# neptune-ai/open-solution-salt-identification

Hardware: AMD Instinct MI355X
Metric: training images/sec, U-Net ResNet34 101x101 (pad->128) bs32/GPU (higher is better)
Workload: dtype bf16; 1 GPU; architectures.unet.UNetResNet(34, hypercolumn) 128x128 (101 resized+edge-padded) batch 32/GPU, lovasz loss, Adam lr1e-4 L2 1e-4, train-mode BN; global_batch=32, parallelism=dp1

## Files before the change

open-solution-salt-identification_amd/csrc/conv_ws.hip:

```cpp
#include <type_traits>
#include "common.h"

#ifndef SALT_LS_D1
#define SALT_LS_D1 4
#endif
#ifndef SALT_LS_NLW
#define SALT_LS_NLW 4
#endif
#ifndef SALT_LS_PREFETCH
#define SALT_LS_PREFETCH 1
#endif
#ifndef SALT_LS_ABLATE
#define SALT_LS_ABLATE 0
#endif
#ifndef SALT_WS_CLK
#define SALT_WS_CLK 0
#endif

namespace {

struct WsKP {
    const bf16_t* x; const bf16_t* w; bf16_t* y;
    const float* bias; const float* scale; const float* shift;
    int B, H, W, x_cs, y_cs, OH, OW;
    int yH, yW, fold_top, ox_shift;
    int Cout, n_tiles, slots;
    int tiles_x, tiles_y, ntiles, per_xcd;
    int min_dy, min_dx, pad_mode;
    int tap_off[9];
    int relu, accumulate;
    const bf16_t* bnb_y; const bf16_t* bnb_a; int bnb_cs, bnb_acs, bnb_relu;
    const float* bnb_mean; const float* bnb_invstd; const float* bnb_gamma; const float* bnb_beta;
    double* fin_acc;
    double* bnb_acc;
    const bf16_t* res; int res_cs;
    long long y_plane;
};

__device__ __attribute__((aligned(16))) unsigned int g_ws_zero[4] = {0u, 0u, 0u, 0u};
#if SALT_WS_CLK
__device__ unsigned long long g_ws_clk[256 * 48];
#endif

typedef __attribute__((address_space(3))) void* lds_ptr_t;
typedef const __attribute__((address_space(1))) void* glb_ptr_t;

__device__ __forceinline__ int ws_swz(int row, int slot) { return row * 64 + (((slot ^ (row >> 2)) & 3) << 4); }
__device__ __forceinline__ int ws_perm(int m) { return (int)((0x73261540u >> ((m >> 2) * 4)) & 0xfu) * 4 + (m & 3); }

__device__ __forceinline__ int ws_perm_inv(int q) { return (int)((0x74216530u >> ((q >> 2) * 4)) & 0xfu) * 4 + (q & 3); }

template <int N> __device__ __forceinline__ void ws_wait_vm() {
    asm volatile("s_waitcnt vmcnt(%0)" :: "n"(N) : "memory");
}

template <int N, int S> __device__ __forceinline__ void ws_halve(float* v, int l31) {
    const bool up = (l31 >> S) & 1;
#pragma unroll
    for (int i = 0; i < N / 2; ++i) {
        const float keep = up ? v[i + N / 2] : v[i], give = up ? v[i] : v[i + N / 2];
        v[i] = keep + __shfl_xor(give, 1 << S);
    }
}

struct WsEpi {
    bf16_t* y; const bf16_t* bnb_y; const bf16_t* bnb_a;
    int y_cs, bnb_cs, bnb_acs, relu, accumulate, bnb_relu;
    bool has_affine, sums;
    const bf16_t* res; int res_cs;
};
template <int NI> struct WsOps { u32x4 oldv[2][NI][2], yv[2][NI][2], av[2][NI][2]; };
template <int NI, bool OLD>
__device__ __forceinline__ void ws_prefetch_operands(const WsEpi& p, const unsigned (&pix)[2], int n0, int khalf, WsOps<NI>& o) {
#pragma unroll
    for (int j = 0; j < NI; ++j)
#pragma unroll
        for (int i = 0; i < 2; ++i)
#pragma unroll
            for (int gp = 0; gp < 2; ++gp) {
                const unsigned c = n0 + 8 * khalf + 32 * j + 16 * gp;
                if (OLD && p.accumulate) o.oldv[i][j][gp] = *reinterpret_cast<const u32x4*>(p.y + (pix[i] * (unsigned)p.y_cs + c));
                if (OLD && p.res) o.oldv[i][j][gp] = *reinterpret_cast<const u32x4*>(p.res + (pix[i] * (unsigned)p.res_cs + c));
                if (p.sums) {
                    o.yv[i][j][gp] = *reinterpret_cast<const u32x4*>(p.bnb_y + (pix[i] * (unsigned)p.bnb_cs + c));
                    if (p.bnb_a) o.av[i][j][gp] = *reinterpret_cast<const u32x4*>(p.bnb_a + (pix[i] * (unsigned)p.bnb_acs + c));
                }
            }
}

struct WsLaneGeo {
    bool valid[2];
    bool do_right, do_top;
    bool fr_on, ft_on;
    int fr_src0, fr_src1;
    int ft_src0, ft_src1;
};

template <int NI, int MODE, bool FOLD>
__device__ __forceinline__ void ws_epilogue_tile(const WsEpi& p, f32x16 (&acc)[2][NI], const unsigned (&pix)[2], const WsLaneGeo& geo, int n0,
                                                 const float* cst, float (&rs0)[NI][4], float (&rs1)[NI][4], int khalf, int l31,
                                                 const WsOps<NI>* pre = nullptr, bool pre_old = true) {
    typedef bf16_t T;
    constexpr int MI = 2, BN = 32 * NI;
    typedef const __attribute__((address_space(3))) float* cst_lds_t;
    cst_lds_t cst_l = (cst_lds_t)cst + 8 * khalf;
    if (MODE == 2) asm volatile("" : "+v"(cst_l));
#pragma unroll
    for (int j = 0; j < NI; ++j) {
        u32x4 oldv[MI][2], yv[MI][2], av[MI][2];
        auto load_operands = [&](int i) {
            if (!geo.valid[i]) return;
            if (pre) {
#pragma unroll
                for (int gp = 0; gp < 2; ++gp) {
                    if (pre_old) oldv[i][gp] = pre->oldv[i][j][gp];
                    else if (p.accumulate) oldv[i][gp] = *reinterpret_cast<const u32x4*>(p.y + (pix[i] * (unsigned)p.y_cs + n0 + 8 * khalf + 32 * j + 16 * gp));
                    yv[i][gp] = pre->yv[i][j][gp]; av[i][gp] = pre->av[i][j][gp];
                }
                return;
            }
            if (MODE != 1 && p.accumulate) {
#pragma unroll
                for (int gp = 0; gp < 2; ++gp)
                    oldv[i][gp] = *reinterpret_cast<const u32x4*>(p.y + (pix[i] * (unsigned)p.y_cs + n0 + 8 * khalf + 32 * j + 16 * gp));
            }
            if (MODE == 0 && p.res) {
#pragma unroll
                for (int gp = 0; gp < 2; ++gp)
                    oldv[i][gp] = *reinterpret_cast<const u32x4*>(p.res + (pix[i] * (unsigned)p.res_cs + n0 + 8 * khalf + 32 * j + 16 * gp));
            }
            if (MODE == 2 && p.sums) {
#pragma unroll
                for (int gp = 0; gp < 2; ++gp) {
                    yv[i][gp] = *reinterpret_cast<const u32x4*>(p.bnb_y + (pix[i] * (unsigned)p.bnb_cs + n0 + 8 * khalf + 32 * j + 16 * gp));
                    if (p.bnb_a) av[i][gp] = *reinterpret_cast<const u32x4*>(p.bnb_a + (pix[i] * (unsigned)p.bnb_acs + n0 + 8 * khalf + 32 * j + 16 * gp));
                }
            }
        };
        if (!FOLD) {
#pragma unroll
            for (int i = 0; i < MI; ++i) load_operands(i);
        }
        float v[MI][16];
#pragma unroll
        for (int i = 0; i < MI; ++i) {
#pragma unroll
            for (int r = 0; r < 16; ++r) v[i][r] = acc[i][j][r];
            if (MODE != 2 && p.has_affine) {
#pragma unroll
                for (int q = 0; q < 4; ++q) {
                    const int ch0 = 32 * j + 8 * q + 4 * khalf;
                    const f32x4 bi = *reinterpret_cast<const f32x4*>(cst + ch0), sc = *reinterpret_cast<const f32x4*>(cst + BN + ch0),
                                sh = *reinterpret_cast<const f32x4*>(cst + 2 * BN + ch0);
#pragma unroll
                    for (int e = 0; e < 4; ++e) {
                        float t = (v[i][4 * q + e] + bi[e]) * sc[e] + sh[e];
                        if (p.relu && !(MODE == 0 && p.res)) t = fmaxf(t, 0.f);
                        v[i][4 * q + e] = t;
                    }
                }
            }
        }
        if (FOLD) {
            const int hb = khalf << 5;
            if (geo.do_right) {
#pragma unroll
                for (int i = 0; i < MI; ++i)
#pragma unroll
                    for (int r = 0; r < 16; ++r) {
                        const float add = __shfl(v[i][r], hb + geo.fr_src0) + __shfl(v[i][r], hb + geo.fr_src1);
                        if (geo.fr_on) v[i][r] += add;
                    }
            }
            if (geo.do_top) {
#pragma unroll
                for (int r = 0; r < 16; ++r) {
                    const float add = __shfl(v[0][r], hb + geo.ft_src0) + __shfl(v[0][r], hb + geo.ft_src1);
                    if (geo.ft_on) v[1][r] += add;
                }
            }
        }
        float t0[16], t1[16];
#pragma unroll
        for (int e = 0; e < 16; ++e) { t0[e] = 0.f; t1[e] = 0.f; }
#pragma unroll
        for (int i = 0; i < MI; ++i) {
            const unsigned yo = pix[i] * (unsigned)p.y_cs + n0 + 8 * khalf + 32 * j;
            if (FOLD) load_operands(i);
            if (MODE == 1) {
#pragma unroll
                for (int r = 0; r < 16; ++r) { t0[r] += v[i][r]; t1[r] += v[i][r] * v[i][r]; }
            }
#pragma unroll
            for (int gp = 0; gp < 2; ++gp) {
                const unsigned ax = f2bf_pk(v[i][8 * gp + 0], v[i][8 * gp + 1]), ay = f2bf_pk(v[i][8 * gp + 2], v[i][8 * gp + 3]);
                const unsigned bx = f2bf_pk(v[i][8 * gp + 4], v[i][8 * gp + 5]), by = f2bf_pk(v[i][8 * gp + 6], v[i][8 * gp + 7]);
                const auto rx = __builtin_amdgcn_permlane32_swap(ax, bx, false, false);
                const auto ry = __builtin_amdgcn_permlane32_swap(ay, by, false, false);
                u32x4 stored = {rx[0], ry[0], rx[1], ry[1]};
                if (!geo.valid[i]) continue;
                if (MODE != 1 && p.accumulate) {
                    float f8[8], o8[8];
                    unpack16<T>(stored, f8); unpack16<T>(oldv[i][gp], o8);
#pragma unroll
                    for (int e = 0; e < 8; ++e) f8[e] += o8[e];
                    stored = pack16<T>(f8);
                }
                if (MODE == 0 && p.res) {
                    float f8[8], o8[8];
                    unpack16<T>(stored, f8); unpack16<T>(oldv[i][gp], o8);
#pragma unroll
                    for (int e = 0; e < 8; ++e) { f8[e] += o8[e]; if (p.relu) f8[e] = fmaxf(f8[e], 0.f); }
                    stored = pack16<T>(f8);
                }
                *reinterpret_cast<u32x4*>(p.y + (yo + 16 * gp)) = stored;
                if (MODE == 2 && p.sums) {
                    const int ch0 = 32 * j + 16 * gp;
                    const cst_lds_t cl = cst_l;
                    float mu[8], is[8], gq[8], yc[8];
                    *reinterpret_cast<f32x4*>(mu) = *reinterpret_cast<const __attribute__((address_space(3))) f32x4*>(cl + ch0);
                    *reinterpret_cast<f32x4*>(mu + 4) = *reinterpret_cast<const __attribute__((address_space(3))) f32x4*>(cl + ch0 + 4);
                    *reinterpret_cast<f32x4*>(is) = *reinterpret_cast<const __attribute__((address_space(3))) f32x4*>(cl + BN + ch0);
                    *reinterpret_cast<f32x4*>(is + 4) = *reinterpret_cast<const __attribute__((address_space(3))) f32x4*>(cl + BN + ch0 + 4);
                    unpack16<T>(stored, gq); unpack16<T>(yv[i][gp], yc);
                    if (p.bnb_a) {
                        float a8[8];
                        unpack16<T>(av[i][gp], a8);
#pragma unroll
                        for (int e = 0; e < 8; ++e) {
                            const float gg = (!p.bnb_relu || a8[e] > 0.f) ? gq[e] : 0.f;
                            t0[gp * 8 + e] += gg; t1[gp * 8 + e] += gg * (yc[e] - mu[e]) * is[e];
                        }
                    } else {
                        float ks[8], sh[8];
                        *reinterpret_cast<f32x4*>(ks) = *reinterpret_cast<const __attribute__((address_space(3))) f32x4*>(cl + 2 * BN + ch0);
                        *reinterpret_cast<f32x4*>(ks + 4) = *reinterpret_cast<const __attribute__((address_space(3))) f32x4*>(cl + 2 * BN + ch0 + 4);
                        *reinterpret_cast<f32x4*>(sh) = *reinterpret_cast<const __attribute__((address_space(3))) f32x4*>(cl + 3 * BN + ch0);
                        *reinterpret_cast<f32x4*>(sh + 4) = *reinterpret_cast<const __attribute__((address_space(3))) f32x4*>(cl + 3 * BN + ch0 + 4);
#pragma unroll
                        for (int e = 0; e < 8; ++e) {
                            const float gg = (!p.bnb_relu || yc[e] * ks[e] + sh[e] > 0.f) ? gq[e] : 0.f;
                            t0[gp * 8 + e] += gg; t1[gp * 8 + e] += gg * (yc[e] - mu[e]) * is[e];
                        }
                    }
                }
            }
        }
        if (MODE != 0 && p.sums) {
            ws_halve<16, 0>(t0, l31); ws_halve<8, 1>(t0, l31);
            ws_halve<16, 0>(t1, l31); ws_halve<8, 1>(t1, l31);
#pragma unroll
            for (int e = 0; e < 4; ++e) { rs0[j][e] += t0[e]; rs1[j][e] += t1[e]; }
        }
    }
}

template <int NI, int MODE, int NW>
__device__ __forceinline__ void ws_sums_flush(float (&rs0)[NI][4], float (&rs1)[NI][4], bool holder, int hw, float* red, int n0, int C,
                                              double* fin_acc, double* bnb_acc, double count, int khalf, int l31) {
    constexpr int BN = 32 * NI;
    const int tid = threadIdx.x;
    const int idx = 8 * (l31 & 1) + 4 * ((l31 >> 1) & 1) + 2 * ((l31 >> 2) & 1) + ((l31 >> 3) & 1);
    if (holder) {
#pragma unroll
        for (int j = 0; j < NI; ++j) {
            ws_halve<4, 2>(rs0[j], l31); ws_halve<2, 3>(rs0[j], l31);
            ws_halve<4, 2>(rs1[j], l31); ws_halve<2, 3>(rs1[j], l31);
            const float s0 = rs0[j][0] + __shfl_xor(rs0[j][0], 16), s1 = rs1[j][0] + __shfl_xor(rs1[j][0], 16);
            const int ch = MODE == 1 ? 32 * j + (idx & 3) + 8 * (idx >> 2) + 4 * khalf : 32 * j + 16 * (idx >> 3) + 8 * khalf + (idx & 7);
            red[(hw * 2 + 0) * BN + ch] = s0;
            red[(hw * 2 + 1) * BN + ch] = s1;
        }
    }
    __syncthreads();
    if (tid < 2 * BN) {
        const int st = tid / BN, n = tid - st * BN;
        double t = 0.0;
#pragma unroll
        for (int w = 0; w < NW; ++w) t += (double)red[(w * 2 + st) * BN + n];
        if (MODE == 1) {
            double* a = fin_acc + (blockIdx.x & 7) * (2 * C + 1);
            fin_add(a + st * C + n0 + n, t);
            if (tid == 0 && count > 0.0) fin_add(a + 2 * C, count);
        } else {
            fin_add(bnb_acc + ((blockIdx.x & 7) * 2 + st) * C + n0 + n, t);
        }
    }
}

template <int NCH, int NI, int MODE, bool FOLD>
__global__ __launch_bounds__(512) void conv_ws_kernel(WsKP p) {
    typedef bf16_t T;
    constexpr int BN = 32 * NI, NT = 9, MI = 2;
    constexpr int HPC = 21;
    constexpr int HP = NCH * HPC;
    constexpr int WP = NCH * NT * BN / 16;
    constexpr int NSW = (WP + 7) / 8;
    constexpr int NSH = (HP + 3) / 4;
    constexpr int W_BYTES = WP * 1024, H_BYTES = HP * 1024, HC_BYTES = HPC * 1024;
    constexpr int OFF_H = W_BYTES, OFF_DUMMY = OFF_H + 2 * H_BYTES;
    constexpr int OFF_CONST = OFF_DUMMY + 1024;
    extern __shared__ __attribute__((aligned(16))) unsigned char smem[];

    const int tid = threadIdx.x, lane = tid & 63;
    const int wave = __builtin_amdgcn_readfirstlane(tid >> 6);
    const int grp = wave >> 2, wm = wave & 3;
    const int khalf = lane >> 5, l31 = lane & 31;

    const int xcd = blockIdx.x & 7, jwg = blockIdx.x >> 3;
    const int nt = jwg % p.n_tiles, slot = jwg / p.n_tiles, n0 = nt * BN;
    const int t_lo = xcd * p.per_xcd;
    const int t_hi = min(t_lo + p.per_xcd, p.ntiles);
    const int n_my = (t_lo + slot < t_hi) ? (t_hi - t_lo - slot + p.slots - 1) / p.slots : 0;
    if (n_my <= 0) return;
    auto tile_of = [&](int k) { return t_lo + slot + k * p.slots; };
    struct TC { int b, oy0, ox0; };
    auto coords = [&](int t) {
        TC c; const int tx = t % p.tiles_x; const int r = t / p.tiles_x;
        c.ox0 = (tx << 4) - p.ox_shift; c.oy0 = (r % p.tiles_y) << 4; c.b = r / p.tiles_y; return c;
    };
#if SALT_WS_CLK
    unsigned long long clk[24]; int nclk = 0;
    auto stamp = [&]() { if (nclk < 22) clk[nclk++] = __builtin_readcyclecounter(); };
#else
    auto stamp = [&]() {};
#endif
    stamp();

    const unsigned char* zp = reinterpret_cast<const unsigned char*>(g_ws_zero);
    auto dma = [&](const void* src, int dst) {
        __builtin_amdgcn_global_load_lds((glb_ptr_t)src, (lds_ptr_t)(smem + dst), 16, 0, 0);
    };
    auto issue_weights = [&]() {
#pragma unroll
        for (int i = 0; i < NSW; ++i) {
            const int q = wave + 8 * i;
            const bool real = q < WP;
            const int R = q * 16 + (lane >> 2);
            const int ct = R / BN, n = R - ct * BN;
            const int cslot = (lane ^ (R >> 2)) & 3;
            const unsigned char* src = real ? reinterpret_cast<const unsigned char*>(p.w + ((ct * p.Cout + n0 + n) * 32 + cslot * 8)) : zp;
            dma(src, real ? q * 1024 : OFF_DUMMY);
        }
    };
    auto issue_halo = [&](const TC& c, int g) {
        int ln = lane;
        asm volatile("" : "+v"(ln));
        const T* xb = p.x + (int64_t)c.b * p.H * p.W * p.x_cs;
        const int iy0 = c.oy0 + p.min_dy, ix0 = c.ox0 + p.min_dx;
        const bool clamp = p.pad_mode != 0;
#pragma unroll
        for (int i = 0; i < NSH; ++i) {
            const int pidx = wm + 4 * i;
            const bool real = pidx < HP;
            const int ch = (NCH > 1 && pidx >= HPC) ? 1 : 0;
            const int row = (pidx - ch * HPC) * 16 + (ln >> 2);
            const int hy = (int)__umulhi((unsigned)row, 238609295u);
            const int hx = row - hy * 18;
            const int iy = iy0 + hy, ix = ix0 + hx;
            const int iyc = min(max(iy, 0), p.H - 1), ixc = min(max(ix, 0), p.W - 1);
            const bool inside = ((unsigned)iy < (unsigned)p.H) & ((unsigned)ix < (unsigned)p.W);
            const bool valid = real & (row < 324) & (clamp | inside);
            const int slot = (ln ^ (row >> 2)) & 3;
            const unsigned char* src = reinterpret_cast<const unsigned char*>(xb + ((iyc * p.W + ixc) * p.x_cs + ch * 32 + slot * 8));
            dma(valid ? src : zp, real ? OFF_H + g * H_BYTES + pidx * 1024 : OFF_DUMMY);
        }
    };

    issue_weights();
    if (grp < n_my) issue_halo(coords(tile_of(grp)), grp);
    if (tid < BN) {
        float* sc = reinterpret_cast<float*>(smem + OFF_CONST);
        if (MODE == 2) {
            if (p.bnb_acc) {
                const float mu = p.bnb_mean[n0 + tid], is = p.bnb_invstd[n0 + tid], k = p.bnb_gamma[n0 + tid] * is;
                sc[tid] = mu; sc[BN + tid] = is; sc[2 * BN + tid] = k; sc[3 * BN + tid] = p.bnb_beta[n0 + tid] - mu * k;
            }
        } else {
            sc[tid] = p.bias ? p.bias[n0 + tid] : 0.f; sc[BN + tid] = p.scale ? p.scale[n0 + tid] : 1.f; sc[2 * BN + tid] = p.shift ? p.shift[n0 + tid] : 0.f;
        }
    }

    int pbase[MI];
#pragma unroll
    for (int i = 0; i < MI; ++i) {
        const int m = wm * 64 + i * 32 + ws_perm(l31);
        pbase[i] = (m >> 4) * 18 + (m & 15);
    }
    f32x16 acc[MI][NI];
    struct Frag { u32x4 a[MI], b[NI]; };
    auto mma_tile = [&](int g) {
        const unsigned char* hb = smem + OFF_H + g * H_BYTES;
        int a_addr[NT][MI], b_addr[NI];
#pragma unroll
        for (int i = 0; i < MI; ++i) {
            int pb = pbase[i];
            asm volatile("" : "+v"(pb));
#pragma unroll
            for (int t = 0; t < NT; ++t) a_addr[t][i] = ws_swz(pb + p.tap_off[t], khalf);
        }
        {
            int lb = l31;
            asm volatile("" : "+v"(lb));
#pragma unroll
            for (int j = 0; j < NI; ++j) b_addr[j] = ws_swz(j * 32 + lb, khalf);
        }
#pragma unroll
        for (int i = 0; i < MI; ++i)
#pragma unroll
            for (int j = 0; j < NI; ++j)
#pragma unroll
                for (int r = 0; r < 16; ++r) acc[i][j][r] = 0.f;
        auto load_frag = [&](int s, Frag& f) {
            const int c = s / (2 * NT), t = (s % (2 * NT)) >> 1, hx = (s & 1) << 5;
#pragma unroll
            for (int i = 0; i < MI; ++i) f.a[i] = *reinterpret_cast<const u32x4*>(hb + c * HC_BYTES + (a_addr[t][i] ^ hx));
#pragma unroll
            for (int j = 0; j < NI; ++j) f.b[j] = *reinterpret_cast<const u32x4*>(smem + (c * NT + t) * (BN * 64) + (b_addr[j] ^ hx));
        };
        auto mma_frag = [&](const Frag& f) {
#pragma unroll
            for (int i = 0; i < MI; ++i)
#pragma unroll
                for (int j = 0; j < NI; ++j)
                    acc[i][j] = __builtin_amdgcn_mfma_f32_32x32x16_bf16(__builtin_bit_cast(bf16x8, f.b[j]), __builtin_bit_cast(bf16x8, f.a[i]), acc[i][j], 0, 0, 0);
        };
        constexpr int NST = NCH * NT * 2;
        Frag f[3];
        load_frag(0, f[0]);
        load_frag(1, f[1]);
        __builtin_amdgcn_sched_group_barrier(0x100, 2 * (MI + NI), 0);
#pragma unroll
        for (int s = 0; s < NST; ++s) {
            if (s + 2 < NST) load_frag(s + 2, f[(s + 2) % 3]);
            mma_frag(f[s % 3]);
            if (s + 2 < NST) __builtin_amdgcn_sched_group_barrier(0x100, MI + NI, 0);
            __builtin_amdgcn_sched_group_barrier(0x008, MI * NI, 0);
        }
    };

    float rs0[NI][4], rs1[NI][4];
#pragma unroll
    for (int j = 0; j < NI; ++j)
#pragma unroll
        for (int e = 0; e < 4; ++e) { rs0[j][e] = 0.f; rs1[j][e] = 0.f; }
    const bool sums = (MODE == 1 && p.fin_acc) || (MODE == 2 && p.bnb_acc);
    const WsEpi ep = {p.y_plane ? p.y + ((long long)nt * p.y_plane - n0) : p.y, p.bnb_y, p.bnb_a, p.y_cs, p.bnb_cs, p.bnb_acs, p.relu, p.accumulate, p.bnb_relu,
                      p.bias || p.scale || p.shift || p.relu, sums, p.res, p.res_cs};

    auto epilogue = [&](const TC& c, int g, bool has_next, const TC& next) {
        unsigned pix[MI];
        WsLaneGeo geo = {{true, true}, false, false, false, false, 0, 0, 0, 0};
#pragma unroll
        for (int i = 0; i < MI; ++i) {
            const int m = wm * 64 + i * 32 + ws_perm(l31);
            const int oy = c.oy0 + (m >> 4), ox = c.ox0 + (m & 15);
            const int iy = oy - p.fold_top;
            geo.valid[i] = ((unsigned)iy < (unsigned)p.yH) & ((unsigned)ox < (unsigned)p.yW);
            pix[i] = (unsigned)((c.b * p.yH + iy) * p.yW + ox);
        }
        if (FOLD) {
            const int q = ws_perm(l31), rs = q >> 4, col = q & 15;
            geo.fr_src0 = ws_perm_inv(rs * 16 + 14); geo.fr_src1 = ws_perm_inv(rs * 16 + 15);
            geo.ft_src0 = ws_perm_inv(col); geo.ft_src1 = ws_perm_inv(16 + col);
            geo.do_right = c.ox0 + 16 == p.OW;
            geo.do_top = wm == 0 && c.oy0 == 0;
            geo.fr_on = col == 13 && geo.do_right;
            geo.ft_on = rs == 0 && geo.do_top;
        }
        ws_epilogue_tile<NI, MODE, FOLD>(ep, acc, pix, geo, n0, reinterpret_cast<const float*>(smem + OFF_CONST), rs0, rs1, khalf, l31);
        stamp();
        if (has_next) {
            __builtin_amdgcn_sched_barrier(0);
            issue_halo(next, g);
        }
    };

    for (int k = 0; k <= n_my; ++k) {
        const int g_mma = k & 1;
        if (k == 0) { if (grp == 0 || n_my < 2) ws_wait_vm<0>(); else ws_wait_vm<NSH>(); }
        else if (grp == g_mma && k < n_my) ws_wait_vm<0>();
        asm volatile("s_waitcnt lgkmcnt(0)" ::: "memory");
        __builtin_amdgcn_s_barrier();
        asm volatile("" ::: "memory");
        stamp();
        if (grp == g_mma) {
            if (k < n_my) { __builtin_amdgcn_s_setprio(1); mma_tile(g_mma); __builtin_amdgcn_s_setprio(0); }
        } else if (k >= 1) {
            const bool has_next = k + 1 < n_my;
            const TC cur = coords(tile_of(k - 1));
            const TC nxt = has_next ? coords(tile_of(k + 1)) : cur;
            epilogue(cur, grp, has_next, nxt);
        }
        stamp();
    }

    if (MODE != 0 && sums) {
        asm volatile("s_waitcnt vmcnt(0)" ::: "memory");
        __syncthreads();
        ws_sums_flush<NI, MODE, 8>(rs0, rs1, true, wave, reinterpret_cast<float*>(smem), n0, p.Cout, p.fin_acc, p.bnb_acc,
                                   nt == 0 ? (double)n_my * 256.0 : 0.0, khalf, l31);
    }
#if SALT_WS_CLK
    if (lane == 0 && (wave == 0 || wave == 4) && blockIdx.x < 256) {
        unsigned long long* o = g_ws_clk + (blockIdx.x * 2 + grp) * 24;
        for (int i = 0; i < 22; ++i) o[i] = i < nclk ? clk[i] : 0ull;
        o[22] = (unsigned long long)n_my;
        o[23] = __builtin_readcyclecounter();
    }
#endif
}


int ws_cus() {
    static int cus = 0;
    if (!cus) {
        hipDeviceProp_t pr; int dev = 0;
        if (hipGetDevice(&dev) == hipSuccess && hipGetDeviceProperties(&pr, dev) == hipSuccess) cus = pr.multiProcessorCount;
        if (cus < 8) cus = 256;
    }
    return cus;
}

template <int NCH, int NI, int MODE, bool FOLD>
int ws_launch_mode(const WsKP& k, hipStream_t st) {
    constexpr int BN = 32 * NI, HP = NCH * 21, WP = NCH * 9 * BN / 16;
    constexpr int LDS = WP * 1024 + 2 * HP * 1024 + 1024 + 4 * BN * 4;
    static_assert(LDS <= 160 * 1024 && 8 * 2 * BN * 4 <= WP * 1024, "LDS budget");
    return salt_launch(conv_ws_kernel<NCH, NI, MODE, FOLD>, dim3((unsigned)(k.slots * k.n_tiles * 8)), dim3(512), LDS, st, k);
}

template <int NCH, int NI>
int ws_launch(const WsKP& k, hipStream_t st) {
    const bool fold = k.fold_top != 0;
    if (k.fin_acc) return ws_launch_mode<NCH, NI, 1, false>(k, st);
    if (k.bnb_acc) return fold ? ws_launch_mode<NCH, NI, 2, true>(k, st) : ws_launch_mode<NCH, NI, 2, false>(k, st);
    return fold ? ws_launch_mode<NCH, NI, 0, true>(k, st) : ws_launch_mode<NCH, NI, 0, false>(k, st);
}

struct LsKP {
    const bf16_t* x; const bf16_t* w; bf16_t* y;
    const float* bias; const float* scale; const float* shift;
    int B, H, W, x_cs, y_cs, OH, OW, Cout;
    int tiles_x, tiles_y, ntiles, per_xcd, n_tiles, slots, nchunk;
    int min_dy, min_dx, pad_mode;
    int tap_off[9];
    int relu, accumulate;
    const bf16_t* bnb_y; const bf16_t* bnb_a; int bnb_cs, bnb_acs, bnb_relu;
    const float* bnb_mean; const float* bnb_invstd; const float* bnb_gamma; const float* bnb_beta;
    double* fin_acc; double* bnb_acc;
    const bf16_t* res; int res_cs;
    long long x_plane;
};

template <int NI, int MODE, int NLW = SALT_LS_NLW, int MT = 1>
__global__ __launch_bounds__(256 + 64 * NLW) void conv_ls_kernel(LsKP p) {
    typedef bf16_t T;
    constexpr int BN = 32 * NI, NT = 9, MI = 2;
    constexpr int HPC = 21, WPC = NT * BN / 16, PC = MT * HPC + WPC;
    constexpr int NS = (PC + NLW - 1) / NLW;
    constexpr int D = NI == 1 ? SALT_LS_D1 : 2;
    constexpr int HT_BYTES = HPC * 1024, H_BYTES = MT * HT_BYTES, CH_BYTES = PC * 1024;
    static_assert(MT == 1 || (MODE == 0 && NI == 2), "two-tile items: plain epilogue, 64-channel blocks");
    constexpr int OFF_DUMMY = D * CH_BYTES, OFF_CONST = OFF_DUMMY + 1024;
    static_assert(OFF_CONST + 4 * BN * 4 <= 160 * 1024, "LDS budget");
    extern __shared__ __attribute__((aligned(16))) unsigned char smem[];

    const int tid = threadIdx.x, lane = tid & 63;
    const int wave = __builtin_amdgcn_readfirstlane(tid >> 6);
    const bool loader = wave >= 4;
    const int wm = wave & 3;
    const int lw = wave - 4;
    const int khalf = lane >> 5, l31 = lane & 31;

    const int xcd = blockIdx.x & 7, jwg = blockIdx.x >> 3;
    if (jwg >= p.slots * p.n_tiles) return;
    const int nt = jwg % p.n_tiles, slot = jwg / p.n_tiles, n0 = nt * BN;
    const int t_lo = xcd * p.per_xcd;
    const int t_hi = min(t_lo + p.per_xcd, p.ntiles);
    const int n_my = (t_lo + slot < t_hi) ? (t_hi - t_lo - slot + p.slots - 1) / p.slots : 0;
    const int n_items = (n_my + MT - 1) / MT;
    if (n_items <= 0) return;
    const int G = n_items * p.nchunk;
    struct TC { int b, oy0, ox0; };
    auto coords = [&](int k) {
        const int t = t_lo + slot + k * p.slots;
        TC c; const int tx = t % p.tiles_x; const int r = t / p.tiles_x;
        c.ox0 = tx << 4; c.oy0 = (r % p.tiles_y) << 4; c.b = r / p.tiles_y; return c;
    };
    if (tid < BN) {
        float* sc = reinterpret_cast<float*>(smem + OFF_CONST);
        if (MODE == 2) {
            if (p.bnb_acc) {
                const float mu = p.bnb_mean[n0 + tid], is = p.bnb_invstd[n0 + tid], k = p.bnb_gamma[n0 + tid] * is;
                sc[tid] = mu; sc[BN + tid] = is; sc[2 * BN + tid] = k; sc[3 * BN + tid] = p.bnb_beta[n0 + tid] - mu * k;
            }
        } else {
            sc[tid] = p.bias ? p.bias[n0 + tid] : 0.f; sc[BN + tid] = p.scale ? p.scale[n0 + tid] : 1.f; sc[2 * BN + tid] = p.shift ? p.shift[n0 + tid] : 0.f;
        }
    }
    asm volatile("s_waitcnt lgkmcnt(0)" ::: "memory");

    float rs0[NI][4], rs1[NI][4];
#pragma unroll
    for (int j = 0; j < NI; ++j)
#pragma unroll
        for (int e = 0; e < 4; ++e) { rs0[j][e] = 0.f; rs1[j][e] = 0.f; }
    const bool sums = (MODE == 1 && p.fin_acc) || (MODE == 2 && p.bnb_acc);

    if (loader) {
        const unsigned char* zp = reinterpret_cast<const unsigned char*>(g_ws_zero);
        auto dma = [&](const void* src, int dst) {
            __builtin_amdgcn_global_load_lds((glb_ptr_t)src, (lds_ptr_t)(smem + dst), 16, 0, 0);
        };
        int w_rel[NS], h_off[NS];
#pragma unroll
        for (int i = 0; i < NS; ++i) {
            const int pi = lw + NLW * i;
            w_rel[i] = 0; h_off[i] = -1;
            if (pi >= MT * HPC && pi < PC) {
                const int R = (pi - MT * HPC) * 16 + (lane >> 2);
                const int t = R / BN, n = R - t * BN;
                w_rel[i] = (t * p.Cout + n0 + n) * 32 + ((lane ^ (R >> 2)) & 3) * 8;
            }
        }
        const T* xb = p.x;
        const T* xb1 = p.x;
        auto item_offsets = [&](int k) {
            const bool clamp = p.pad_mode != 0;
            TC cm[MT];
#pragma unroll
            for (int m = 0; m < MT; ++m) cm[m] = coords(MT == 1 ? k : min(MT * k + m, n_my - 1));
            xb = p.x + (int64_t)cm[0].b * p.H * p.W * p.x_cs;
            if (MT == 2) xb1 = p.x + (int64_t)cm[MT - 1].b * p.H * p.W * p.x_cs;
#pragma unroll
            for (int i = 0; i < NS; ++i) {
                const int pi = lw + NLW * i;
                if (pi < MT * HPC) {
                    const int m = MT == 1 ? 0 : (pi >= HPC ? 1 : 0), hp = pi - m * HPC;
                    const TC c = cm[m];
                    const int iy0 = c.oy0 + p.min_dy, ix0 = c.ox0 + p.min_dx;
                    const int row = hp * 16 + (lane >> 2);
                    const int hy = (int)__umulhi((unsigned)row, 238609295u);
                    const int hx = row - hy * 18;
                    const int iy = iy0 + hy, ix = ix0 + hx;
                    const int iyc = min(max(iy, 0), p.H - 1), ixc = min(max(ix, 0), p.W - 1);
                    const bool inside = ((unsigned)iy < (unsigned)p.H) & ((unsigned)ix < (unsigned)p.W);
                    const bool valid = (row < 324) & (clamp | inside) & (MT == 1 || MT * k + m < n_my);
                    h_off[i] = valid ? (iyc * p.W + ixc) * p.x_cs + ((lane ^ (row >> 2)) & 3) * 8 : -1;
                }
            }
        };
        int ik = 0, ic = 0, ig = 0;
        auto issue_next = [&]() {
            const bool live = ig < G;
            if (live && ic == 0) item_offsets(ik);
            const int buf = (ig % D) * CH_BYTES;
            const T* wc = p.w + (int64_t)ic * NT * p.Cout * 32;
            const long long coff = p.x_plane ? (long long)(ic >> 1) * p.x_plane + (ic & 1) * 32 : (long long)ic * 32;
            const T* xc = xb + coff;
            const T* xc1 = xb1 + coff;
#pragma unroll
            for (int i = 0; i < NS; ++i) {
                const int pi = lw + NLW * i;
                const void* src = zp;
                int dst = OFF_DUMMY;
                if (live && pi < MT * HPC) { if (h_off[i] >= 0) src = ((MT == 2 && pi >= HPC) ? xc1 : xc) + h_off[i]; dst = buf + pi * 1024; }
                else if (live && pi < PC) { src = wc + w_rel[i]; dst = buf + pi * 1024; }
                if (!(SALT_LS_ABLATE & 2)) dma(src, dst);
            }
            if (live) { ++ig; if (++ic == p.nchunk) { ic = 0; ++ik; } }
        };
#pragma unroll 1
        for (int d = 0; d < D - 1; ++d) issue_next();
#pragma unroll 1
        for (int g = 0; g < G; ++g) {
            ws_wait_vm<(D - 2) * NS>();
            asm volatile("" ::: "memory");
            __builtin_amdgcn_s_barrier();
            asm volatile("" ::: "memory");
            issue_next();
        }
        ws_wait_vm<0>();
    } else {
        int pbase[MI];
#pragma unroll
        for (int i = 0; i < MI; ++i) {
            const int m = wm * 64 + i * 32 + ws_perm(l31);
            pbase[i] = (m >> 4) * 18 + (m & 15);
        }
        const WsEpi ep = {p.y, p.bnb_y, p.bnb_a, p.y_cs, p.bnb_cs, p.bnb_acs, p.relu, p.accumulate, p.bnb_relu,
                          p.bias || p.scale || p.shift || p.relu, sums, p.res, p.res_cs};
        struct Frag { u32x4 a[MT][MI], b[NI]; };
        int g = 0;
#pragma unroll 1
        for (int k = 0; k < n_items; ++k) {
            f32x16 acc[MT][MI][NI];
#pragma unroll
            for (int m = 0; m < MT; ++m)
#pragma unroll
                for (int i = 0; i < MI; ++i)
#pragma unroll
                    for (int j = 0; j < NI; ++j)
#pragma unroll
                        for (int r = 0; r < 16; ++r) acc[m][i][j][r] = 0.f;
            int a_addr[MT == 1 ? NT : 1][MI], b_addr[NI];
            if constexpr (MT == 1) {
#pragma unroll
                for (int i = 0; i < MI; ++i) {
                    int pb = pbase[i];
                    asm volatile("" : "+v"(pb));
#pragma unroll
                    for (int t = 0; t < NT; ++t) a_addr[t][i] = ws_swz(pb + p.tap_off[t], khalf);
                }
            }
            {
                int lb = l31;
                asm volatile("" : "+v"(lb));
#pragma unroll
                for (int j = 0; j < NI; ++j) b_addr[j] = H_BYTES + ws_swz(j * 32 + lb, khalf);
            }
            unsigned pix[MT][MI];
            auto set_pix = [&](int lx) {
#pragma unroll
                for (int mt = 0; mt < MT; ++mt) {
                    const TC cc = coords(MT == 1 ? k : min(MT * k + mt, n_my - 1));
#pragma unroll
                    for (int i = 0; i < MI; ++i) {
                        const int m = wm * 64 + i * 32 + ws_perm(lx);
                        pix[mt][i] = (unsigned)((cc.b * p.OH + cc.oy0 + (m >> 4)) * p.OW + cc.ox0 + (m & 15));
                    }
                }
            };
            constexpr bool PRE = MODE == 2 && SALT_LS_PREFETCH != 0;
            if (PRE || MT == 1) set_pix(l31);
            WsOps<PRE ? NI : 1> ops;
            constexpr bool PRE_OLD = NI == 1;
            if constexpr (PRE) ws_prefetch_operands<NI, PRE_OLD>(ep, pix[0], n0, khalf, ops);
            __builtin_amdgcn_s_setprio(1);
#pragma unroll 1
            for (int c = 0; c < p.nchunk; ++c, ++g) {
                asm volatile("" ::: "memory");
                __builtin_amdgcn_s_barrier();
                asm volatile("" ::: "memory");
                if (SALT_LS_ABLATE & 1) continue;
                const unsigned char* hb = smem + (g % D) * CH_BYTES;
                int pbc[MI];
#pragma unroll
                for (int i = 0; i < MI; ++i) { pbc[i] = pbase[i]; if (MT != 1) asm volatile("" : "+v"(pbc[i])); }
                auto load_frag = [&](int s, Frag& f) {
                    const int t = s >> 1, hx = (s & 1) << 5;
#pragma unroll
                    for (int i = 0; i < MI; ++i) {
                        const int ad = (MT == 1 ? a_addr[t][i] : ws_swz(pbc[i] + p.tap_off[t], khalf)) ^ hx;
#pragma unroll
                        for (int m = 0; m < MT; ++m) f.a[m][i] = *reinterpret_cast<const u32x4*>(hb + m * HT_BYTES + ad);
                    }
#pragma unroll
                    for (int j = 0; j < NI; ++j) f.b[j] = *reinterpret_cast<const u32x4*>(hb + t * (BN * 64) + (b_addr[j] ^ hx));
                };
                auto mma_frag = [&](const Frag& f) {
#pragma unroll
                    for (int m = 0; m < MT; ++m)
#pragma unroll
                        for (int i = 0; i < MI; ++i)
#pragma unroll
                            for (int j = 0; j < NI; ++j)
                                acc[m][i][j] = __builtin_amdgcn_mfma_f32_32x32x16_bf16(__builtin_bit_cast(bf16x8, f.b[j]), __builtin_bit_cast(bf16x8, f.a[m][i]), acc[m][i][j], 0, 0, 0);
                };
                constexpr int NST = NT * 2;
                constexpr int FR = MT == 1 ? 3 : 2;
                Frag f[FR];
                load_frag(0, f[0]);
                if (FR == 3) load_frag(1, f[1]);
                __builtin_amdgcn_sched_group_barrier(0x100, (FR - 1) * (MT * MI + NI), 0);
#pragma unroll
                for (int s2 = 0; s2 < NST; ++s2) {
                    if (s2 + FR - 1 < NST) load_frag(s2 + FR - 1, f[(s2 + FR - 1) % FR]);
                    mma_frag(f[s2 % FR]);
                    if (s2 + FR - 1 < NST) __builtin_amdgcn_sched_group_barrier(0x100, MT * MI + NI, 0);
                    __builtin_amdgcn_sched_group_barrier(0x008, MT * MI * NI, 0);
                }
            }
            __builtin_amdgcn_s_setprio(0);
            if (!(PRE || MT == 1)) {
                int lx = l31;
                asm volatile("" : "+v"(lx));
                set_pix(lx);
            }
            const WsLaneGeo geo = {{true, true}, false, false, false, false, 0, 0, 0, 0};
// ... 842 lines not shown
```

Baseline: 6444 images/s.

## Prefetch BN-backward epilogue operands ahead of use in warp-specialized conv

In MODE 2, the conv epilogue's operand loads (bnb_y, bnb_a) are now software-pipelined. For NI==1 they are issued before the MMA tile so their latency hides behind the matrix work. For larger NI, the loads for column block j+1 are issued while block j is being processed. Invalid lanes are clamped to a safe pixel address so loads can be issued unconditionally. The cost is higher register pressure from holding prefetched operands, which may lower occupancy or cause spills.

New measurement: 6449 images/s, median of 2. Within noise of the previous version (+0.1%).

```diff
diff --git a/open-solution-salt-identification_amd/csrc/conv_ws.hip b/open-solution-salt-identification_amd/csrc/conv_ws.hip
--- a/open-solution-salt-identification_amd/csrc/conv_ws.hip
+++ b/open-solution-salt-identification_amd/csrc/conv_ws.hip
@@ -9,6 +9,9 @@
 #endif
 #ifndef SALT_LS_PREFETCH
 #define SALT_LS_PREFETCH 1
+#endif
+#ifndef SALT_WS_PREFETCH
+#define SALT_WS_PREFETCH 1
 #endif
 #ifndef SALT_LS_ABLATE
 #define SALT_LS_ABLATE 0
@@ -99,47 +102,53 @@
 template <int NI, int MODE, bool FOLD>
 __device__ __forceinline__ void ws_epilogue_tile(const WsEpi& p, f32x16 (&acc)[2][NI], const unsigned (&pix)[2], const WsLaneGeo& geo, int n0,
                                                  const float* cst, float (&rs0)[NI][4], float (&rs1)[NI][4], int khalf, int l31,
-                                                 const WsOps<NI>* pre = nullptr, bool pre_old = true) {
+                                                 const WsOps<NI>* pre = nullptr, bool pre_old = true, const unsigned (*fpix)[2] = nullptr) {
     typedef bf16_t T;
     constexpr int MI = 2, BN = 32 * NI;
     typedef const __attribute__((address_space(3))) float* cst_lds_t;
     cst_lds_t cst_l = (cst_lds_t)cst + 8 * khalf;
     if (MODE == 2) asm volatile("" : "+v"(cst_l));
+    const bool piped = MODE == 2 && fpix != nullptr;
+    u32x4 oldv[MI][2], yv[MI][2], av[MI][2];
+    auto load_operands = [&](int j, int i) {
+        if (!piped && !geo.valid[i]) return;
+        if (pre) {
+#pragma unroll
+            for (int gp = 0; gp < 2; ++gp) {
+                if (pre_old) oldv[i][gp] = pre->oldv[i][j][gp];
+                else if (p.accumulate) oldv[i][gp] = *reinterpret_cast<const u32x4*>(p.y + (pix[i] * (unsigned)p.y_cs + n0 + 8 * khalf + 32 * j + 16 * gp));
+                yv[i][gp] = pre->yv[i][j][gp]; av[i][gp] = pre->av[i][j][gp];
+            }
+            return;
+        }
+        const unsigned px = piped ? (*fpix)[i] : pix[i];
+        if (MODE != 1 && p.accumulate) {
+#pragma unroll
+            for (int gp = 0; gp < 2; ++gp)
+                oldv[i][gp] = *reinterpret_cast<const u32x4*>(p.y + (px * (unsigned)p.y_cs + n0 + 8 * khalf + 32 * j + 16 * gp));
+        }
+        if (MODE == 0 && p.res) {
+#pragma unroll
+            for (int gp = 0; gp < 2; ++gp)
+                oldv[i][gp] = *reinterpret_cast<const u32x4*>(p.res + (px * (unsigned)p.res_cs + n0 + 8 * khalf + 32 * j + 16 * gp));
+        }
+        if (MODE == 2 && p.sums) {
+#pragma unroll
+            for (int gp = 0; gp < 2; ++gp) {
+                yv[i][gp] = *reinterpret_cast<const u32x4*>(p.bnb_y + (px * (unsigned)p.bnb_cs + n0 + 8 * khalf + 32 * j + 16 * gp));
+                if (p.bnb_a) av[i][gp] = *reinterpret_cast<const u32x4*>(p.bnb_a + (px * (unsigned)p.bnb_acs + n0 + 8 * khalf + 32 * j + 16 * gp));
+            }
+        }
+    };
+    if (piped) {
+#pragma unroll
+        for (int i = 0; i < MI; ++i) load_operands(0, i);
+    }
 #pragma unroll
     for (int j = 0; j < NI; ++j) {
-        u32x4 oldv[MI][2], yv[MI][2], av[MI][2];
-        auto load_operands = [&](int i) {
-            if (!geo.valid[i]) return;
-            if (pre) {
-#pragma unroll
-                for (int gp = 0; gp < 2; ++gp) {
-                    if (pre_old) oldv[i][gp] = pre->oldv[i][j][gp];
-                    else if (p.accumulate) oldv[i][gp] = *reinterpret_cast<const u32x4*>(p.y + (pix[i] * (unsigned)p.y_cs + n0 + 8 * khalf + 32 * j + 16 * gp));
-                    yv[i][gp] = pre->yv[i][j][gp]; av[i][gp] = pre->av[i][j][gp];
-                }
-                return;
-            }
-            if (MODE != 1 && p.accumulate) {
-#pragma unroll
-                for (int gp = 0; gp < 2; ++gp)
-                    oldv[i][gp] = *reinterpret_cast<const u32x4*>(p.y + (pix[i] * (unsigned)p.y_cs + n0 + 8 * khalf + 32 * j + 16 * gp));
-            }
-            if (MODE == 0 && p.res) {
-#pragma unroll
-                for (int gp = 0; gp < 2; ++gp)
-                    oldv[i][gp] = *reinterpret_cast<const u32x4*>(p.res + (pix[i] * (unsigned)p.res_cs + n0 + 8 * khalf + 32 * j + 16 * gp));
-            }
-            if (MODE == 2 && p.sums) {
-#pragma unroll
-                for (int gp = 0; gp < 2; ++gp) {
-                    yv[i][gp] = *reinterpret_cast<const u32x4*>(p.bnb_y + (pix[i] * (unsigned)p.bnb_cs + n0 + 8 * khalf + 32 * j + 16 * gp));
-                    if (p.bnb_a) av[i][gp] = *reinterpret_cast<const u32x4*>(p.bnb_a + (pix[i] * (unsigned)p.bnb_acs + n0 + 8 * khalf + 32 * j + 16 * gp));
-                }
-            }
-        };
-        if (!FOLD) {
-#pragma unroll
-            for (int i = 0; i < MI; ++i) load_operands(i);
+        if (!piped && !FOLD) {
+#pragma unroll
+            for (int i = 0; i < MI; ++i) load_operands(j, i);
         }
         float v[MI][16];
 #pragma unroll
@@ -186,7 +195,7 @@
 #pragma unroll
         for (int i = 0; i < MI; ++i) {
             const unsigned yo = pix[i] * (unsigned)p.y_cs + n0 + 8 * khalf + 32 * j;
-            if (FOLD) load_operands(i);
+            if (!piped && FOLD) load_operands(j, i);
             if (MODE == 1) {
 #pragma unroll
                 for (int r = 0; r < 16; ++r) { t0[r] += v[i][r]; t1[r] += v[i][r] * v[i][r]; }
@@ -245,6 +254,7 @@
                     }
                 }
             }
+            if (piped && j + 1 < NI) load_operands(j + 1, i);
         }
         if (MODE != 0 && p.sums) {
             ws_halve<16, 0>(t0, l31); ws_halve<8, 1>(t0, l31);
@@ -448,17 +458,31 @@
     const WsEpi ep = {p.y_plane ? p.y + ((long long)nt * p.y_plane - n0) : p.y, p.bnb_y, p.bnb_a, p.y_cs, p.bnb_cs, p.bnb_acs, p.relu, p.accumulate, p.bnb_relu,
                       p.bias || p.scale || p.shift || p.relu, sums, p.res, p.res_cs};
 
-    auto epilogue = [&](const TC& c, int g, bool has_next, const TC& next) {
-        unsigned pix[MI];
-        WsLaneGeo geo = {{true, true}, false, false, false, false, 0, 0, 0, 0};
+    auto lane_pixels = [&](const TC& c, unsigned (&pix)[MI], bool (&valid)[MI]) {
 #pragma unroll
         for (int i = 0; i < MI; ++i) {
             const int m = wm * 64 + i * 32 + ws_perm(l31);
             const int oy = c.oy0 + (m >> 4), ox = c.ox0 + (m & 15);
             const int iy = oy - p.fold_top;
-            geo.valid[i] = ((unsigned)iy < (unsigned)p.yH) & ((unsigned)ox < (unsigned)p.yW);
+            valid[i] = ((unsigned)iy < (unsigned)p.yH) & ((unsigned)ox < (unsigned)p.yW);
             pix[i] = (unsigned)((c.b * p.yH + iy) * p.yW + ox);
         }
+    };
+    constexpr bool PRE = MODE == 2 && SALT_WS_PREFETCH != 0;
+    constexpr bool PRE_EARLY = PRE && NI == 1;
+    auto fetch_pixels = [&](const TC& c, unsigned (&pix)[MI]) {
+        bool valid[MI];
+        lane_pixels(c, pix, valid);
+        const unsigned first = (unsigned)((c.b * p.yH + max(c.oy0 - p.fold_top, 0)) * p.yW + max(c.ox0, 0));
+#pragma unroll
+        for (int i = 0; i < MI; ++i) pix[i] = valid[i] ? pix[i] : first;
+    };
+    WsOps<PRE_EARLY ? NI : 1> early;
+
+    auto epilogue = [&](const TC& c, int g, bool has_next, const TC& next) {
+        unsigned pix[MI];
+        WsLaneGeo geo = {{true, true}, false, false, false, false, 0, 0, 0, 0};
+        lane_pixels(c, pix, geo.valid);
         if (FOLD) {
             const int q = ws_perm(l31), rs = q >> 4, col = q & 15;
             geo.fr_src0 = ws_perm_inv(rs * 16 + 14); geo.fr_src1 = ws_perm_inv(rs * 16 + 15);
@@ -468,7 +492,13 @@
             geo.fr_on = col == 13 && geo.do_right;
             geo.ft_on = rs == 0 && geo.do_top;
         }
-        ws_epilogue_tile<NI, MODE, FOLD>(ep, acc, pix, geo, n0, reinterpret_cast<const float*>(smem + OFF_CONST), rs0, rs1, khalf, l31);
+        const float* cst = reinterpret_cast<const float*>(smem + OFF_CONST);
+        if constexpr (PRE_EARLY) ws_epilogue_tile<NI, MODE, FOLD>(ep, acc, pix, geo, n0, cst, rs0, rs1, khalf, l31, &early);
+        else if constexpr (PRE) {
+            unsigned fpix[MI];
+            fetch_pixels(c, fpix);
+            ws_epilogue_tile<NI, MODE, FOLD>(ep, acc, pix, geo, n0, cst, rs0, rs1, khalf, l31, nullptr, true, &fpix);
+        } else ws_epilogue_tile<NI, MODE, FOLD>(ep, acc, pix, geo, n0, cst, rs0, rs1, khalf, l31);
         stamp();
         if (has_next) {
             __builtin_amdgcn_sched_barrier(0);
@@ -485,7 +515,14 @@
         asm volatile("" ::: "memory");
         stamp();
         if (grp == g_mma) {
-            if (k < n_my) { __builtin_amdgcn_s_setprio(1); mma_tile(g_mma); __builtin_amdgcn_s_setprio(0); }
+            if (k < n_my) {
+                if constexpr (PRE_EARLY) {
+                    unsigned fpix[MI];
+                    fetch_pixels(coords(tile_of(k)), fpix);
+                    ws_prefetch_operands<NI, true>(ep, fpix, n0, khalf, early);
+                }
+                __builtin_amdgcn_s_setprio(1); mma_tile(g_mma); __builtin_amdgcn_s_setprio(0);
+            }
         } else if (k >= 1) {
             const bool has_next = k + 1 < n_my;
             const TC cur = coords(tile_of(k - 1));
```
